# weimengmeng1999/AdapterSIS

Hardware: AMD Instinct MI355X
Metric: training images/sec, ViT-L/14 588^2 adapter fine-tune (higher is better)
Workload: dtype f16; 1 GPU; vit_large/14 frozen + CAViT/CACNN adapters (n_last_blocks=4) + FeatureDecoder, 588x588, batch 12/GPU, reference_exact train.py step (fwd + decoder bwd + all-reduce + SGD), random-init weights; global_batch=12, image_size=588, parallelism=dp1, split_precision_convs=True, split_attn_out=False, precise_level=0, fold_attn_scale=True, fused_qkv=False, dead_cacnn_elided=True, c1_elided=True, ln_fold=True, mx_conv=True, mx_dense=True, conv_halo=True, fuse_cls_up=False, skipped_optimizer_steps=0

## Files before the change

### adaptersis_amd/_lib.py

```python
from __future__ import annotations

import ctypes as C
import os

_HERE = os.path.dirname(os.path.abspath(__file__))
LIB_PATH = os.path.join(_HERE, "lib", "libasis_hip.so")

ASIS_F16, ASIS_BF16, ASIS_F32 = 0, 1, 2
ASIS_EINVAL, ASIS_ELAUNCH = -1, -2
ACT_NONE, ACT_GELU, ACT_RELU, ACT_SILU_MUL, ACT_GELU_GRAD = 0, 1, 2, 3, 4


class AsisError(RuntimeError):
    pass


class GemmDesc(C.Structure):
    _fields_ = [
        ("A", C.c_void_p), ("B", C.c_void_p), ("C", C.c_void_p),
        ("lda", C.c_int64), ("ldb", C.c_int64), ("ldc", C.c_int64),
        ("strideA", C.c_int64), ("strideB", C.c_int64), ("strideC", C.c_int64),
        ("batch", C.c_int32), ("M", C.c_int32), ("N", C.c_int32), ("K", C.c_int32),
        ("bias_n", C.c_void_p), ("bias_m", C.c_void_p), ("scale_n", C.c_void_p), ("res", C.c_void_p),
        ("ldr", C.c_int64), ("strideR", C.c_int64),
# ... 75 lines not shown
    "asis_dwconv_bwd_nblk": [_i64],
    "asis_dwconv_gelu_bwd": [_vp, _i, _vp, _vp, _vp, _vp, _vp, _i, _vp, _vp, _vp, _vp, _i, _i, _i],
    "asis_rowblock_nblk": [_i64],
    "asis_layernorm_bwd": [_vp, _vp, _i64, _vp, _i64, _vp, _f, _vp, _i64, _vp, _i64, _vp, _i64, _i],
    "asis_gelu16": [_vp, _i, _vp, _vp, _vp, _i64],
    "asis_gelu_split": [_vp, _i, _vp, _vp, _vp, _i64],
    "asis_cast_colsum": [_vp, _i, _vp, _i64, _vp, _i64, _f, _vp, _i64, _i],
    "asis_layernorm_gather": [_vp, _i, _vp, _i64, _vp, _vp, _f, _vp, _i64, _vp, _i, _i, _i64, _i],
    "asis_scaled_index_add": [_vp, _vp, _i64, _vp, _i64, _vp, _i64, _vp, _i, _i, _i64, _i],
    "asis_gather_cast_colsum": [_vp, _i, _vp, _i64, _vp, _i64, _vp, _vp, _i, _i, _i64, _i],
    "asis_layernorm_bwd_scatter": [_vp, _vp, _i64, _vp, _i64, _vp, _f, _vp, _i64, _vp, _i64, _vp, _vp, _i, _i, _i64, _i64, _i],
    "asis_swiglu_bwd": [_vp, _i, _vp, _vp, _vp, _i64, _i],
    "asis_colsum": [_vp, _i, _vp, _i64, _vp, _i64, _i],
    "asis_ls_linear_finish": [_vp, _vp, _vp, _vp, _vp, _vp, _f, _vp, _vp, _vp, _i, _i],
    "asis_attention_fwd": [_vp, _i, _vp, _vp, _i64, _vp, _i64, _vp, _i64, _i, _i, _i, _f],
    "asis_im2col_patch": [_vp, _i, _vp, _i, _i, _i, _i, _vp, _i64],
    "asis_im2col_patch_split": [_vp, _i, _vp, _i, _i, _i, _i, _vp, _vp, _i64],
    "asis_cast_pad": [_vp, _i, _vp, _i64, _vp, _i64, _i64, _i, _f, _i],
    "asis_add_cls_pos": [_vp, _vp, _vp, _vp, _vp, _i, _i, _i],
    "asis_msda_fwd": [_vp, _i, _vp, _vp, _i64, _vp, _vp, _vp, _vp, _i, _i, _i, _i, _i, _i, _i],
    "asis_msda_fwd_split": [_vp, _i, _vp, _vp, _i64, _vp, _vp, _vp, _vp, _vp, _i, _i, _i, _i, _i, _i, _i],
    "asis_dwconv_gelu": [_vp, _i, _vp, _vp, _vp, _vp, _vp, _i, _vp, _i, _i, _i],
    "asis_conv3x3_c3": [_vp, _vp, _vp, _vp, _i, _i, _i, _i, _i, _i],
    "asis_conv3x3_smallcout_fwd": [_vp, _i, _vp, _vp, _vp, _vp, _vp, _i, _i, _i, _i, _i],
    "asis_conv3x3_smallcout_fwd_up": [_vp, _i, _vp, _vp, _vp, _vp, _vp, _vp, _i, _i, _i, _i, _i],
    "asis_conv3x3_smallcout_wgrad_up": [_vp, _i, _vp, _i, _vp, _vp, _vp, _vp, _i, _i, _i, _i, _i, _i],
    "asis_cls_lowres_nblk": [_i, _i, _i],
    "asis_cls_lowres_fwd": [_vp, _vp, _vp, _vp, _vp, _vp, _vp, _vp, _i, _i, _i, _i, _i],
    "asis_cls_lowres_bwd": [_vp, _i, _vp, _vp, _i, _vp, _vp, _vp, _vp, _vp, _vp, _vp, _vp, _vp, _i, _i, _i, _i, _i, _i],
    "asis_dgrad_lowres_nblk": [_i, _i, _i],
    "asis_dgrad_lowres_cap": [_i],
    "asis_dgrad_lowres_pack": [_vp, _i, _vp, _vp, _vp, _i, _i],
    "asis_dgrad_lowres": [_vp, _i, _vp, _vp, _vp, _vp, _vp, _vp, _vp, _vp, _vp, _vp, _vp, _i, _i, _i, _i, _i, _i],
    "asis_conv3x3_smallcout_dgrad": [_vp, _i, _vp, _vp, _i, _vp, _vp, _i, _i, _i, _i, _i],
    "asis_conv3x3_smallcout_wgrad": [_vp, _i, _vp, _i, _vp, _vp, _i, _i, _i, _i, _i, _i],
    "asis_colstats_nparts": [_i64],
    "asis_colstats": [_vp, _vp, _i64, _i, _vp],
    "asis_reduce_partials": [_vp, _vp, _i, _i, _vp],
    "asis_bn_finalize": [_vp, _vp, _d, _i, _vp, _vp, _f, _f, _vp, _vp, _vp, _vp, _vp, _vp, _vp],
    "asis_bn_eval_affine": [_vp, _vp, _vp, _vp, _vp, _f, _i, _vp, _vp],
    "asis_bn_act": [_vp, _i, _vp, _vp, _vp, _i, _vp, _vp, _i64, _i],
    "asis_bn_act_mx": [_vp, _i, _vp, _vp, _vp, _i, _vp, _vp, _vp, _i64, _i],
    "asis_bn_relu_maxpool": [_vp, _i, _vp, _vp, _vp, _vp, _vp, _i, _i, _i, _i],
    "asis_bn_relu_upsample": [_vp, _i, _vp, _vp, _vp, _vp, _vp, _i, _i, _i, _i, _i],
    "asis_pack_conv_weight": [_vp, _i, _vp, _vp, _i, _i, _i, _i, _i, _i64, _i],
    "asis_decoder_input": [_vp, _i, _vp, _i64, _vp, _i64, _vp, _i64, _vp, _vp, _i, _i, _i, _i, _i, _i],
    "asis_swiglu": [_vp, _i, _vp, _vp, _i64, _i],
    "asis_swiglu_split": [_vp, _i, _vp, _vp, _vp, _i64, _i],
    "asis_copy_channels": [_vp, _vp, _i64, _vp, _i64, _i64, _i64],
    "asis_add_f32": [_vp, _vp, _vp, _vp, _i64, _i, _i64, _i64, _i64],
    "asis_maxpool2_fwd": [_vp, _i, _vp, _vp, _vp, _vp, _vp, _i, _i, _i, _i],
    "asis_maxpool2_bwd": [_vp, _vp, _vp, _vp, _i, _i, _i, _i],
    "asis_cls_l2norm": [_vp, _vp, _vp, _vp, _i, _i, _i, _i],
    "asis_cls_l2norm_bwd": [_vp, _vp, _vp, _vp, _vp, _i, _i, _i, _i],
    "asis_mask_logits_fwd": [_vp, _vp, _vp, _vp, _vp, _f, _vp, _vp, _vp, _i, _i, _i, _i],
    "asis_mask_logits_nblk": [_i, _i],
    "asis_mask_logits_bwd": [_vp, _vp, _vp, _vp, _vp, _vp, _vp, _f, _vp, _vp, _vp, _i, _i, _i, _i],
    "asis_mask_dchat": [_vp, _vp, _vp, _vp, _vp, _i, _i, _i, _i],
    "asis_nearest_add_relu": [_vp, _i, _vp, _vp, _vp, _vp, _vp, _vp, _i, _i, _i, _i, _i, _i],
    "asis_nearest_sum": [_vp, _vp, _vp, _vp, _vp, _i, _i, _i, _i, _i, _i],
    "asis_convt2x2_scatter": [_vp, _i, _vp, _vp, _vp, _i, _i, _i, _i, _i, _i, _i, _i, _i, _i],
    "asis_convt2x2_gather": [_vp, _i, _vp, _vp, _vp, _i, _i, _i, _i, _i, _i, _i, _i, _i, _i],
    "asis_convt2x2_bias_nblk": [_i64],
    "asis_conv1x1_dgrad_small": [_vp, _i, _vp, _vp, _i64, _vp, _vp, _i64, _i, _i],
    "asis_convt2x2_bias_grad": [_vp, _vp, _vp, _i, _i, _i, _i, _i, _i, _i, _i, _i, _i],
    "asis_dice_nblk": [_i, _i],
# ... 86 lines not shown
```

### adaptersis_amd/backbones/decoders.py

```python
from __future__ import annotations

import os
from typing import Dict, List, Optional

import torch
import torch.nn as nn
import torch.nn.functional as F

from .. import config, ops, parallel
from ..dinov2.layers.blocks import _Packed, _pack
from . import _bn


_DGRAD_MX = __import__("os").environ.get("ASIS_DGRAD_MX", "1") not in ("0", "")


class _Stage:
    __slots__ = ("x16", "raw", "scale", "shift", "mean", "invstd", "count", "factor", "stride", "pad", "pool", "cls_lowres", "dgrad_lowres")


def _conv_weights(owner: _Packed, key: str, conv: nn.Conv2d, split: bool):
    dt = config.operand_dtype
    if split:
        w_hi, w_lo, _ = _pack(owner._cache, key + ".wpair", conv.weight, lambda p: ops.pack_conv_weight_pair(p.float().contiguous(), 0, dt))
        return w_hi, w_lo
    return _pack(owner._cache, key + ".w", conv.weight, lambda p: ops.pack_conv_weight(p.float().contiguous(), 0, dt)), None


_KSPLIT = os.environ.get("ASIS_CONV_KSPLIT", "1") != "0"


def _conv_ksplit(P: int, Cout: int, Cin: int, split: bool) -> int:
    if not _KSPLIT or Cin % 64 or P < 256 or Cout < 32 or Cout % 4:
        return 1
    cus = 256
    plan = ops.conv3x3_plan(P, Cout, Cin, split)
    if plan and plan[0].startswith("conv_ph8"):
        tiles = plan[1]
        now, cut = -(-tiles // cus), -(-3 * tiles // cus) / 3.0 * 1.08
        return 3 if cut < 0.88 * now else 1
    tiles = ((P + 255) // 256) * ((Cout + 127) // 128 if Cout > 64 else (Cout + 63) // 64)

    def cost(t):
        c = -(-t // cus)
        return 1.7 * (c // 2) + (c % 2)

    now, cut = cost(tiles), cost(3 * tiles) / 3.0 * 1.08
    r = 3 if cut < 0.88 * now else 1
    if r == 3 and os.environ.get("ASIS_CONV_KSPLIT_DEBUG"):
        print(f"[ksplit] P={P} Cout={Cout} Cin={Cin} tiles={tiles} now={now:.2f} cut={cut:.2f}", flush=True)
    return r


def _conv_weights_mx(owner: _Packed, key: str, conv: nn.Conv2d):
    dt = config.operand_dtype
    amax = _w_amax(owner, key, conv)
    return _pack(owner._cache, key + ".wpairmx", conv.weight,
                 lambda p: ops.pack_conv_weight_pair(p.float().contiguous(), 0, dt, mx=True, amax=amax))


def _w_amax(owner: _Packed, key: str, conv: nn.Conv2d):
    return _pack(owner._cache, key + ".wamax", conv.weight, lambda p: ops.conv_weight_absmax(p.float().contiguous()))


def conv_bn_relu_up_forward(owner: _Packed, key: str, x16, x_lo, conv: nn.Conv2d, bn: nn.BatchNorm2d, factor: int,
                            sync_bn: bool, save: bool, training: bool = True, stride: int = 1, pad: int = 1,
                            pool: bool = False, mx_out: bool = False, defer_up: bool = False):
    dt = config.operand_dtype
    split_out = x_lo is not None
    if key in config.unsplit_layers:
        x_lo = None
    split = x_lo is not None
    B, H, W, _ = x16.shape
    OH, OW = (H + 2 * pad - 3) // stride + 1, (W + 2 * pad - 3) // stride + 1
    mx_in = ops.mx_amax_of(x_lo) if split else None
    if mx_in is not None:
        w_hi, w_lo, w_amax = _conv_weights_mx(owner, key, conv)
    else:
        w_hi, w_lo = _conv_weights(owner, key, conv, split)
    bias = owner._f32(key + ".b", conv.bias)
    ks = _conv_ksplit(B * OH * OW, conv.out_channels, x16.shape[3], split)
    stats = torch.empty((ops.gemm_tiles_m(B * OH * OW), 2, conv.out_channels), device=x16.device,
                        dtype=torch.float32) if (training and ks == 1) else None
    if mx_in is not None and ks == 1 and ops.conv_halo_ok(x16, conv.out_channels, stride, pad):
        raw = ops.conv3x3_halo_mx(x16, x_lo, w_hi, w_lo, (mx_in, w_amax), bias_n=bias, want_stats=training)
        if training:
            raw, stats = raw
    elif mx_in is not None:
        raw = ops.conv_gemm_split(x16, x_lo, w_hi, w_lo, 3, 3, stride, pad, bias_n=bias, stats=stats, ksplit=ks, mx=(mx_in, w_amax))
    elif split:
        raw = ops.conv_gemm_split(x16, x_lo, w_hi, w_lo, 3, 3, stride, pad, bias_n=bias, stats=stats, ksplit=ks)
    else:
        raw = ops.conv_gemm(x16, w_hi, 3, 3, stride, pad, bias_n=bias, stats=stats, ksplit=ks)
    if training and ks > 1:
        stats = ops.colstats(raw)
    if training:
        scale, shift, mean, invstd, count = _bn.finalize(stats, B * OH * OW, bn, sync_bn)
    else:
        scale, shift = ops.bn_eval_affine(bn)
        mean = invstd = count = None
        save = False
    if defer_up:
        up = ("deferred", raw, scale, shift)
    elif pool:
        up = ops.bn_relu_maxpool(raw, scale, shift, dt, split_out)
    elif factor > 1 and mx_out and split_out:
        up = ops.bn_relu_upsample(raw, scale, shift, factor, dt, True, mx_amax=ops.bn_relu_absmax(raw, scale, shift))
    elif factor > 1:
        up = ops.bn_relu_upsample(raw, scale, shift, factor, dt, split_out)
    elif mx_out and split_out:
        up = ops.bn_act(raw, scale, shift, True, dt, True, mx_amax=ops.bn_relu_absmax(raw, scale, shift))
    else:
        up = ops.bn_act(raw, scale, shift, True, dt, split_out)
    if not split_out and not defer_up:
        up = (up, None)
    st = None
    if save:
        st = _Stage()
        st.x16, st.raw, st.scale, st.shift, st.mean, st.invstd, st.count, st.factor = \
            x16, raw, scale, shift, mean, invstd, count, factor
        st.stride, st.pad, st.pool = stride, pad, pool
    return up, st


def conv_bn_relu_up_backward(owner: _Packed, key: str, st: _Stage, dU, conv: nn.Conv2d, bn: nn.BatchNorm2d,
                             inv_scale: float, grads: Dict[str, torch.Tensor], prefix: str, need_dx: bool,
                             sync_bn: bool, conv_name: Optional[str] = None, bn_name: Optional[str] = None,
                             lower: Optional[_Stage] = None):
    conv_name = conv_name or prefix + ".0"
    bn_name = bn_name or prefix + ".1"
    import torch.distributed as dist
    dt = config.operand_dtype
    C = conv.out_channels
    stride, pad = getattr(st, "stride", 1) or 1, getattr(st, "pad", 1)
    if isinstance(dU, tuple):
        g, partial = dU
    elif getattr(st, "pool", False):
        g, partial = ops.maxpool_bn_relu_bwd(dU, st.raw, st.scale, st.shift, st.mean, st.invstd)
    else:
        g, partial = ops.upsample_bn_relu_bwd(dU, st.raw, st.scale, st.shift, st.mean, st.invstd, st.factor)
    red = ops.reduce_rows(partial.view(partial.shape[0], 2 * C))
    local = red
    if sync_bn and parallel.bn_collectives_on():
        local = red.clone()
        dist.all_reduce(red)
    dbeta_s, dgamma_s = red[:C], red[C:]
    split = config.split_conv and need_dx
# ... 74 lines not shown
            parallel.join_grad_streams()
        return (None, None) + tuple(grads[n] for n in ctx.names)


class FeatureDecoder(_Packed):
    def __init__(self, img_size=588, inplanes=64, embed_dim=1024, num_classes=2, features=[1024, 512, 256, 128, 64]):
        super().__init__()
        self.img_size, self.features, self.inplanes = img_size, list(features), inplanes
        self.embed_dim, self.num_classes = embed_dim, num_classes
        chans = [features[0] * 3, features[1], features[2], features[3], features[4]]
        for c in chans:
            if c % 8:
                raise ValueError("FeatureDecoder channel counts must be multiples of 8")
        for i in range(4):
            setattr(self, f"decoder_{i + 1}", nn.Sequential(
                nn.Conv2d(chans[i], chans[i + 1], 3, padding=1), nn.BatchNorm2d(chans[i + 1]), nn.ReLU(inplace=True),
                nn.Upsample(scale_factor=2, mode="bilinear", align_corners=True)))
        self.final_out = nn.Conv2d(chans[4], num_classes, 3, padding=1)
        self.sync_bn = False

    GRAD_ORDER = ("final_out", "decoder_4", "decoder_3", "decoder_2", "decoder_1")

    def _to_nhwc16(self, x):
        B, C, H, W = x.shape
        x2 = x.detach().permute(0, 2, 3, 1).contiguous().float().view(B * H * W, C)
        hi = ops.cast_pad(x2, C, config.operand_dtype).view(B, H, W, C)
        lo = ops.cast_pad(x2, C, config.operand_dtype, part=1).view(B, H, W, C) if config.split_conv else None
        return hi, lo

    def _forward_core(self, x16, x_lo, save: bool, training: Optional[bool] = None):
        training = self.training if training is None else training
        saved: List = []
        a = (x16, x_lo)
        for i in range(1, 5):
            seq = getattr(self, f"decoder_{i}")
            nxt = getattr(self, f"decoder_{i + 1}")[0] if i < 4 else None
            Bq, Hq, Wq, _ = a[0].shape
            mx_out = bool(config.mx_conv_on() and a[1] is not None and nxt is not None and f"d{i + 1}" not in config.unsplit_layers and
                          ops.mx_conv_ok(Bq * 4 * Hq * Wq, nxt.in_channels, nxt.out_channels))
            fo = self.final_out
            fuse = bool(i == 4 and a[1] is not None and ops.FUSE_CLS_UP and seq[0].out_channels == 64 and fo.in_channels == 64 and
                        fo.out_channels <= 8 and Hq >= 4 and Wq >= 8)
            lowres = bool(i == 4 and not fuse and ops.CLS_LOWRES and seq[0].out_channels == 64 and fo.in_channels == 64 and
                          2 <= fo.out_channels <= 4 and Hq >= 2 and Wq >= 2)
            defer = fuse or lowres
            a, st = conv_bn_relu_up_forward(self, f"d{i}", a[0], a[1], seq[0], seq[1], 2, self.sync_bn, save, training, mx_out=mx_out,
                                            defer_up=defer)
            if lowres and st is not None:
                st.cls_lowres = True
            saved.append(st)
        if isinstance(a[0], str):
            if lowres:
                logits = ops.cls_lowres_fwd(a[1], a[2], a[3], self._f32("final.wf", self.final_out.weight),
                                            self._f32("final.b", self.final_out.bias))
            else:
                logits = ops.conv3x3_smallcout_fwd_up(a[1], a[2], a[3], self._f32("final.wf", self.final_out.weight),
                                                      self._f32("final.b", self.final_out.bias), config.operand_dtype)
            saved.append(None)
            return logits, saved
        logits = self._final_forward(a)
        saved.append(a[0] if save else None)
        return logits, saved

    def _final_forward(self, a):
        bias = self._f32("final.b", self.final_out.bias)
        fo = self.final_out
        if fo.out_channels <= 16 and fo.in_channels in (8, 16, 32, 64):
            return ops.conv3x3_smallcout_fwd(a[0], a[1], self._f32("final.wf", fo.weight), bias)
        w_hi, w_lo = _conv_weights(self, "final", self.final_out, a[1] is not None)
        if a[1] is not None:
            return ops.conv_gemm_split(a[0], a[1], w_hi, w_lo, 3, 3, 1, 1, bias_n=bias)
        return ops.conv_gemm(a[0], w_hi, 3, 3, 1, 1, bias_n=bias)

    def _final_backward(self, x5, d16, d_lo, bias_partial, inv_scale, grads, dlogits_f32, st4=None):
        C = self.num_classes
        if bias_partial is not None:
            ops.reduce_rows(bias_partial, inv_scale, grads["final_out.bias"])
        else:
            ops.reduce_rows(dlogits_f32, 1.0, grads["final_out.bias"])
        wout = grads["final_out.weight"]
        if x5 is None and getattr(st4, "cls_lowres", False):
            g, partial, slabs = ops.cls_lowres_bwd(d16, d_lo, st4.raw, st4.scale, st4.shift, st4.mean, st4.invstd,
                                                   self._f32("final.wf", self.final_out.weight), reduce=False)
# ... 314 lines not shown
```

### adaptersis_amd/config.py

```python
import os

import torch

operand_dtype = torch.bfloat16 if os.environ.get("ASIS_OPERAND", "f16").lower() in ("bf16", "bfloat16") else torch.float16
loss_scale = float(os.environ.get("ASIS_LOSS_SCALE", 65536.0 if operand_dtype == torch.float16 else 1.0))


def set_operand_dtype(dt: torch.dtype) -> None:
    global operand_dtype
    if dt not in (torch.float16, torch.bfloat16):
        raise ValueError("operand dtype must be float16 or bfloat16")
    operand_dtype = dt

split_conv = os.environ.get("ASIS_SPLIT_CONV", "1") != "0"

precise_attention = os.environ.get("ASIS_PRECISE", "0") not in ("0", "")
fold_attn_scale = os.environ.get("ASIS_FOLD_SCALE", "1") not in ("0", "")
fused_qkv = os.environ.get("ASIS_FUSED_QKV", "0") not in ("0", "")

encoder_stream = os.environ.get("ASIS_ENC_STREAM", "1") not in ("0", "")

vt_stream = os.environ.get("ASIS_VT_STREAM", "1") not in ("0", "")

wgrad_stream = os.environ.get("ASIS_WGRAD_STREAM", "1") not in ("0", "")
# ... 33 lines not shown

_mx = os.environ.get("ASIS_MX_CONV", "1")
mx_conv_all = _mx == "2"
mx_conv = _mx not in ("0", "")


def mx_conv_on() -> bool:
    return mx_conv and (mx_conv_all or operand_dtype == torch.float16)


mx_dense = os.environ.get("ASIS_MX_DENSE", "1") not in ("0", "")


def mx_dense_on() -> bool:
    return mx_dense and operand_dtype == torch.float16

_DGRAD_LOWRES_ALL = ("d2", "d3", "d4")


def parse_dgrad_lowres(v: str) -> frozenset:
    v = (v or "").strip().lower()
    if v in ("", "0"):
        return frozenset()
    if v == "1":
        return frozenset(_DGRAD_LOWRES_ALL)
    keys = [k.strip() for k in v.split(",") if k.strip()]
    bad = [k for k in keys if k not in _DGRAD_LOWRES_ALL]
    if bad:
        raise ValueError(f"ASIS_DGRAD_LOWRES={v!r}: expected 0, 1 or a list of {', '.join(_DGRAD_LOWRES_ALL)} (unknown: {', '.join(bad)})")
    return frozenset(keys)


dgrad_lowres = parse_dgrad_lowres(os.environ.get("ASIS_DGRAD_LOWRES", "1"))
```

### adaptersis_amd/csrc/core.hip

```cpp
#include <stdarg.h>

#include "asis_common.h"

static thread_local char g_err[512] = "";

extern "C" void asis_set_error_(const char* fmt, ...) {
  va_list ap;
  va_start(ap, fmt);
  vsnprintf(g_err, sizeof(g_err), fmt, ap);
  va_end(ap);
}

extern "C" const char* asis_last_error(void) { return g_err; }
extern "C" int asis_version(void) { return 100; }

extern "C" int asis_device_count(void) {
  int n = 0;
  hipError_t e = hipGetDeviceCount(&n);
  if (e != hipSuccess) {
    asis_set_error_("hipGetDeviceCount: %s", hipGetErrorString(e));
    (void)hipGetLastError();
    return ASIS_ELAUNCH;
  }
  return n;
}
```

### adaptersis_amd/ops.py

```python
from __future__ import annotations

import ctypes as C
import functools
import os
from typing import Optional

import torch

from . import _lib, config
from ._lib import ACT_GELU, ACT_GELU_GRAD, ACT_NONE, ACT_RELU, ACT_SILU_MUL, GemmDesc, check, lib

T16_DEFAULT = torch.float16

PROFILE = None


def _launch_timed(kind: str, flops: float, fn, nbytes: float = 0.0):
    if PROFILE is None:
        return fn()
    s, e = torch.cuda.Event(enable_timing=True), torch.cuda.Event(enable_timing=True)
    s.record()
    rc = fn()
    e.record()
    PROFILE.append((kind, flops, s, e, nbytes))
# ... 833 lines not shown

def dgrad_lowres_pack(w: torch.Tensor, dtype: torch.dtype):
    _dev(w)
    Co, Ck = w.shape[0], w.shape[1]
    if w.dtype != torch.float32 or not w.is_contiguous() or tuple(w.shape[2:]) != (3, 3):
        raise ValueError("dgrad_lowres_pack: contiguous float32 [Co, Ck, 3, 3] expected")
    hi = torch.empty((max(Co // 16, 1), 5, Ck, 32), device=w.device, dtype=dtype)
    lo = torch.empty_like(hi)
    check(lib().asis_dgrad_lowres_pack(_stream(), _dt(dtype), w.data_ptr(), hi.data_ptr(), lo.data_ptr(), Co, Ck),
          "asis_dgrad_lowres_pack")
    return hi, lo


def dgrad_lowres(d16: torch.Tensor, d_lo: Optional[torch.Tensor], wpack, raw: torch.Tensor, scale, shift, mean, invstd):
    _dev(d16, d_lo, raw)
    _not_mx("dgrad_lowres", d_lo)
    B, H, W, Ck = raw.shape
    Co = d16.shape[3]
    w_hi, w_lo = wpack
    if not d16.is_contiguous() or tuple(d16.shape[:3]) != (B, 2 * H, 2 * W) or (d_lo is not None and
                                                                                 (d_lo.shape != d16.shape or not d_lo.is_contiguous())):
        raise ValueError("dgrad_lowres: d16 / d_lo must be contiguous [B, 2H, 2W, Co]")
    if raw.dtype != torch.float32 or not raw.is_contiguous() or w_hi.dtype != d16.dtype or w_hi.numel() != (Co // 16) * 5 * Ck * 32:
        raise ValueError("dgrad_lowres: raw must be contiguous float32 [B, H, W, Ck] and the weight pack that of a [Co, Ck, 3, 3] conv")
    nblk = lib().asis_dgrad_lowres_nblk(B, H, W)
    g = torch.empty_like(raw)
    partial = torch.empty((nblk, 2, Ck), device=raw.device, dtype=torch.float32)
    check(lib().asis_dgrad_lowres(_stream(), _dt(d16.dtype), d16.data_ptr(), _p(d_lo), w_hi.data_ptr(), w_lo.data_ptr(), raw.data_ptr(),
                                  _f32c(scale).data_ptr(), _f32c(shift).data_ptr(), _f32c(mean).data_ptr(), _f32c(invstd).data_ptr(),
                                  g.data_ptr(), partial.data_ptr(), nblk, B, H, W, Co, Ck), "asis_dgrad_lowres")
    return g, partial


def conv3x3_smallcout_dgrad(dy_hi: torch.Tensor, dy_lo: Optional[torch.Tensor], w: torch.Tensor) -> torch.Tensor:
    _dev(dy_hi, dy_lo, w)
    B, H, W, CoP = dy_hi.shape
    Cout, Cin = w.shape[0], w.shape[1]
    dx = torch.empty((B, H, W, Cin), device=dy_hi.device, dtype=torch.float32)
    check(lib().asis_conv3x3_smallcout_dgrad(_stream(), _dt(dy_hi.dtype), dy_hi.data_ptr(), _p(dy_lo), CoP,
                                             _f32c(w).data_ptr(), dx.data_ptr(), B, H, W, Cin, Cout),
          "asis_conv3x3_smallcout_dgrad")
    return dx


def colstats(x: torch.Tensor) -> torch.Tensor:
    _dev(x)
    Cc = x.shape[-1]
    R = x.numel() // Cc
    nparts = lib().asis_colstats_nparts(R)
    partial = torch.empty((nparts, 2, Cc), device=x.device, dtype=torch.float32)
    check(lib().asis_colstats(_stream(), _f32c(x).data_ptr(), R, Cc, partial.data_ptr()), "asis_colstats")
    return partial


def reduce_partials(partial: torch.Tensor) -> torch.Tensor:
    _dev(partial)
    nparts, _, Cc = partial.shape
    sums = torch.empty((2, Cc), device=partial.device, dtype=torch.float64)
    check(lib().asis_reduce_partials(_stream(), _f32c(partial).data_ptr(), nparts, Cc, sums.data_ptr()),
          "asis_reduce_partials")
    return sums


def bn_finalize(sums: torch.Tensor, count: float, gamma, beta, eps: float, momentum: float, running_mean=None,
                running_var=None, num_batches_tracked=None):
    _dev(sums, gamma, beta, running_mean, running_var, num_batches_tracked)
# ... 1604 lines not shown
```

### include/asis_hip.h

```cpp
#ifndef ASIS_HIP_H
#define ASIS_HIP_H

#include <stdint.h>

#ifdef __cplusplus
extern "C" {
#endif

#define ASIS_OK 0
#define ASIS_EINVAL (-1)
#define ASIS_ELAUNCH (-2)

#define ASIS_F16 0
#define ASIS_BF16 1
#define ASIS_F32 2

#define ASIS_ACT_NONE 0
#define ASIS_ACT_GELU 1
#define ASIS_ACT_RELU 2
#define ASIS_ACT_SILU_MUL 3
#define ASIS_ACT_GELU_GRAD 4

const char* asis_last_error(void);
int asis_version(void);
// ... 131 lines not shown
                              const int32_t* shapes, const int32_t* starts, void* ST, int64_t ldt, int B, int Lq, int Lin,
                              int M, int L, int P);
int asis_dwconv_bwd_nblk(int64_t rows);
int asis_dwconv_gelu_bwd(void* stream, int dtype, const float* x, const float* w9, const float* bias, const int32_t* shapes,
                         const int32_t* starts, int L, const float* dy, float* g, float* partial, void* dx, int B, int Ntok,
                         int C);

int asis_conv3x3_c3(void* stream, const float* img, const float* w, float* out, int B, int H, int W, int Cout,
                    int stride, int pad);
int asis_conv3x3_smallcout_fwd(void* stream, int dtype, const void* x_hi, const void* x_lo, const float* w,
                               const float* bias, float* out, int B, int H, int W, int Cin, int Cout);
int asis_conv3x3_smallcout_dgrad(void* stream, int dtype, const void* dy_hi, const void* dy_lo, int CoP, const float* w,
                                 float* dx, int B, int H, int W, int Cin, int Cout);

int asis_conv3x3_smallcout_fwd_up(void* stream, int dtype, const float* raw, const float* scale, const float* shift, const float* w,
                                  const float* bias, float* out, int B, int H, int W, int Cin, int Cout);
int asis_conv3x3_smallcout_wgrad_up(void* stream, int dtype, const void* dy, int CoP, const float* raw, const float* scale,
                                    const float* shift, float* slabs, int nblk, int B, int H, int W, int Cin, int Cout);

int asis_cls_lowres_nblk(int B, int H, int W);
int asis_cls_lowres_fwd(void* stream, const float* raw, const float* scale, const float* shift, const float* w, const float* bias,
                        float* z, float* out, int B, int H, int W, int Cin, int Cout);
int asis_cls_lowres_bwd(void* stream, int dtype, const void* d16, const void* d_lo, int CoP, const float* raw, const float* scale,
                        const float* shift, const float* mean, const float* invstd, const float* w, float* g, float* partial,
                        float* slabs, int nblk, int B, int H, int W, int Cin, int Cout);

int asis_dgrad_lowres_nblk(int B, int H, int W);
int asis_dgrad_lowres_cap(int cap);
int asis_dgrad_lowres_pack(void* stream, int dtype, const float* w, void* w_hi, void* w_lo, int Co, int Ck);
int asis_dgrad_lowres(void* stream, int dtype, const void* d16, const void* d_lo, const void* w_hi, const void* w_lo, const float* raw,
                      const float* scale, const float* shift, const float* mean, const float* invstd, float* g, float* partial,
                      int nblk, int B, int H, int W, int Co, int Ck);

int asis_conv3x3_smallcout_wgrad(void* stream, int dtype, const void* dy, int CoP, const void* x, float* slabs, int nblk,
                                 int B, int H, int W, int Cin, int Cout);
int asis_colstats_nparts(int64_t R);
int asis_colstats(void* stream, const float* x, int64_t R, int C, float* partial);
int asis_reduce_partials(void* stream, const float* partial, int nparts, int C, double* sums);
int asis_bn_finalize(void* stream, const double* sums, double count, int C, const float* gamma, const float* beta,
                     float eps, float momentum, float* running_mean, float* running_var, int64_t* num_batches_tracked,
                     float* scale, float* shift, float* mean_out, float* invstd_out);
int asis_bn_eval_affine(void* stream, const float* gamma, const float* beta, const float* running_mean,
                        const float* running_var, float eps, int C, float* scale, float* shift);
int asis_bn_act(void* stream, int dtype, const float* x, const float* scale, const float* shift, int relu, void* out,
                void* out_lo, int64_t R, int C);
int asis_bn_act_mx(void* stream, int dtype, const float* x, const float* scale, const float* shift, int relu, void* out, void* out_mx,
                   const float* amax, int64_t R, int C);
int asis_bn_relu_maxpool(void* stream, int dtype, const float* x, const float* scale, const float* shift, void* out,
                         void* out_lo, int B, int H, int W, int C);
int asis_bn_relu_upsample(void* stream, int dtype, const float* x, const float* scale, const float* shift, void* out,
                          void* out_lo, int B, int H, int W, int C, int factor);
int asis_bn_relu_upsample_mx(void* stream, int dtype, const float* x, const float* scale, const float* shift, void* out,
                             void* out_mx, const float* amax, int B, int H, int W, int C, int factor);
int asis_pack_conv_weight(void* stream, int dtype, const float* w, void* out, int Cout, int Cin, int KH, int KW,
                          int mode, int64_t ldo, int part);
int asis_pack_conv_weight_mx(void* stream, int dtype, const float* w, void* out_mx, int Cout, int Cin, int KH, int KW,
                             int mode, int64_t ldo, const float* amax);
int asis_pack_conv_weight_pair(void* stream, int dtype, const float* w, void* out_hi, void* out_lo, int Cout, int Cin, int KH,
                               int KW, int mode, int64_t ldo, const float* amax);
int asis_decoder_input(void* stream, int dtype, const float* xs, int64_t xs_bstride, const float* c4,
                       int64_t c4_bstride, const float* vit, int64_t vit_bstride, void* out, void* out_lo, int B, int h,
                       int w, int h4, int w4, int D);
int asis_decoder_input_mx(void* stream, int dtype, const float* xs, int64_t xs_bstride, const float* c4, int64_t c4_bstride,
                          const float* vit, int64_t vit_bstride, void* out, void* out_mx, const float* amax, int B, int h,
                          int w, int h4, int w4, int D);
int asis_swiglu(void* stream, int dtype, const float* x12, void* out, int64_t R, int Hd);
// ... 184 lines not shown
```

Baseline: 232.1 img/s.

## Run decoder conv at low resolution before bilinear upsample for d2/d3

For decoder stages d2 and d3, the 3x3 conv no longer runs on the 2x bilinearly upsampled map. Instead the previous stage emits its low-resolution BN+ReLU output, a split-precision GEMM computes all 9 taps at low resolution into a [B,H,W,9,Co] buffer, and a new gather kernel applies the align-corners bilinear upsample per tap, adds the bias and accumulates BN statistics. This cuts the conv GEMM work about fourfold and avoids materialising the upsampled input. The cost is a large fp32 intermediate of 9*Co values per low-res pixel, plus an upsampled copy still built when activations are saved for backward. Zero-padding at the high-res borders is handled by skipping out-of-range taps.

```diff
diff --git a/adaptersis_amd/_lib.py b/adaptersis_amd/_lib.py
--- a/adaptersis_amd/_lib.py
+++ b/adaptersis_amd/_lib.py
@@ -131,6 +131,9 @@
     "asis_dgrad_lowres_cap": [_i],
     "asis_dgrad_lowres_pack": [_vp, _i, _vp, _vp, _vp, _i, _i],
     "asis_dgrad_lowres": [_vp, _i, _vp, _vp, _vp, _vp, _vp, _vp, _vp, _vp, _vp, _vp, _vp, _i, _i, _i, _i, _i, _i],
+    "asis_conv_lowres_tiles": [_i, _i, _i],
+    "asis_conv_lowres_pack": [_vp, _i, _vp, _vp, _vp, _i, _i],
+    "asis_conv_lowres_gather": [_vp, _vp, _vp, _vp, _vp, _i, _i, _i, _i, _i],
     "asis_conv3x3_smallcout_dgrad": [_vp, _i, _vp, _vp, _i, _vp, _vp, _i, _i, _i, _i, _i],
     "asis_conv3x3_smallcout_wgrad": [_vp, _i, _vp, _i, _vp, _vp, _i, _i, _i, _i, _i, _i],
     "asis_colstats_nparts": [_i64],
diff --git a/adaptersis_amd/backbones/decoders.py b/adaptersis_amd/backbones/decoders.py
--- a/adaptersis_amd/backbones/decoders.py
+++ b/adaptersis_amd/backbones/decoders.py
@@ -16,7 +16,7 @@
 
 
 class _Stage:
-    __slots__ = ("x16", "raw", "scale", "shift", "mean", "invstd", "count", "factor", "stride", "pad", "pool", "cls_lowres", "dgrad_lowres")
+    __slots__ = ("x16", "raw", "scale", "shift", "mean", "invstd", "count", "factor", "stride", "pad", "pool", "cls_lowres", "dgrad_lowres", "conv_lowres")
 
 
 def _conv_weights(owner: _Packed, key: str, conv: nn.Conv2d, split: bool):
@@ -65,8 +65,20 @@
 
 def conv_bn_relu_up_forward(owner: _Packed, key: str, x16, x_lo, conv: nn.Conv2d, bn: nn.BatchNorm2d, factor: int,
                             sync_bn: bool, save: bool, training: bool = True, stride: int = 1, pad: int = 1,
-                            pool: bool = False, mx_out: bool = False, defer_up: bool = False):
+                            pool: bool = False, mx_out: bool = False, defer_up: bool = False, low_out: bool = False):
     dt = config.operand_dtype
+    if isinstance(x16, tuple):
+        _, y_hi, y_lo = x16
+        x16 = x_lo
+        wp = _pack(owner._cache, key + ".wlowres", conv.weight, lambda p: ops.conv_lowres_pack(p.float().contiguous(), dt))
+        raw = ops.conv_lowres_fwd(y_hi, y_lo, wp, owner._f32(key + ".b", conv.bias), want_stats=training)
+        stats = None
+        if training:
+            raw, stats = raw
+        up, st = _bn_relu_out(raw, stats, x16, True, bn, factor, sync_bn, save, training, 1, 1, False, mx_out, defer_up, low_out)
+        if st is not None:
+            st.conv_lowres = True
+        return up, st
     split_out = x_lo is not None
     if key in config.unsplit_layers:
         x_lo = None
@@ -94,14 +106,23 @@
         raw = ops.conv_gemm(x16, w_hi, 3, 3, stride, pad, bias_n=bias, stats=stats, ksplit=ks)
     if training and ks > 1:
         stats = ops.colstats(raw)
+    return _bn_relu_out(raw, stats, x16, split_out, bn, factor, sync_bn, save, training, stride, pad, pool, mx_out, defer_up, low_out)
+
+
+def _bn_relu_out(raw, stats, x16, split_out: bool, bn: nn.BatchNorm2d, factor: int, sync_bn: bool, save: bool, training: bool,
+                 stride: int, pad: int, pool: bool, mx_out: bool, defer_up: bool, low_out: bool):
+    dt = config.operand_dtype
     if training:
-        scale, shift, mean, invstd, count = _bn.finalize(stats, B * OH * OW, bn, sync_bn)
+        scale, shift, mean, invstd, count = _bn.finalize(stats, raw.numel() // raw.shape[3], bn, sync_bn)
     else:
         scale, shift = ops.bn_eval_affine(bn)
         mean = invstd = count = None
         save = False
     if defer_up:
         up = ("deferred", raw, scale, shift)
+    elif low_out:
+        y_hi, y_lo = ops.bn_act(raw, scale, shift, True, dt, True)
+        up = (("lowres", y_hi, y_lo), ops.bn_relu_upsample(raw, scale, shift, factor, dt, False) if save else None)
     elif pool:
         up = ops.bn_relu_maxpool(raw, scale, shift, dt, split_out)
     elif factor > 1 and mx_out and split_out:
@@ -112,7 +133,7 @@
         up = ops.bn_act(raw, scale, shift, True, dt, True, mx_amax=ops.bn_relu_absmax(raw, scale, shift))
     else:
         up = ops.bn_act(raw, scale, shift, True, dt, split_out)
-    if not split_out and not defer_up:
+    if not split_out and not defer_up and not low_out:
         up = (up, None)
     st = None
     if save:
@@ -253,23 +274,28 @@
         training = self.training if training is None else training
         saved: List = []
         a = (x16, x_lo)
+        split = x_lo is not None
+        Bq, Hq, Wq, _ = x16.shape
         for i in range(1, 5):
             seq = getattr(self, f"decoder_{i}")
             nxt = getattr(self, f"decoder_{i + 1}")[0] if i < 4 else None
-            Bq, Hq, Wq, _ = a[0].shape
-            mx_out = bool(config.mx_conv_on() and a[1] is not None and nxt is not None and f"d{i + 1}" not in config.unsplit_layers and
+            mx_out = bool(config.mx_conv_on() and split and nxt is not None and f"d{i + 1}" not in config.unsplit_layers and
                           ops.mx_conv_ok(Bq * 4 * Hq * Wq, nxt.in_channels, nxt.out_channels))
             fo = self.final_out
-            fuse = bool(i == 4 and a[1] is not None and ops.FUSE_CLS_UP and seq[0].out_channels == 64 and fo.in_channels == 64 and
+            fuse = bool(i == 4 and split and ops.FUSE_CLS_UP and seq[0].out_channels == 64 and fo.in_channels == 64 and
                         fo.out_channels <= 8 and Hq >= 4 and Wq >= 8)
             lowres = bool(i == 4 and not fuse and ops.CLS_LOWRES and seq[0].out_channels == 64 and fo.in_channels == 64 and
                           2 <= fo.out_channels <= 4 and Hq >= 2 and Wq >= 2)
             defer = fuse or lowres
-            a, st = conv_bn_relu_up_forward(self, f"d{i}", a[0], a[1], seq[0], seq[1], 2, self.sync_bn, save, training, mx_out=mx_out,
-                                            defer_up=defer)
+            low_out = bool(nxt is not None and split and f"d{i + 1}" not in config.unsplit_layers and
+                           ops.conv_lowres_on(f"d{i + 1}") and nxt.in_channels == seq[0].out_channels and
+                           ops.conv_lowres_ok(nxt.out_channels, nxt.in_channels, Hq, Wq))
+            a, st = conv_bn_relu_up_forward(self, f"d{i}", a[0], a[1], seq[0], seq[1], 2, self.sync_bn, save, training,
+                                            mx_out=mx_out and not low_out, defer_up=defer, low_out=low_out)
             if lowres and st is not None:
                 st.cls_lowres = True
             saved.append(st)
+            Hq, Wq = 2 * Hq, 2 * Wq
         if isinstance(a[0], str):
             if lowres:
                 logits = ops.cls_lowres_fwd(a[1], a[2], a[3], self._f32("final.wf", self.final_out.weight),
diff --git a/adaptersis_amd/config.py b/adaptersis_amd/config.py
--- a/adaptersis_amd/config.py
+++ b/adaptersis_amd/config.py
@@ -89,3 +89,21 @@
 
 
 dgrad_lowres = parse_dgrad_lowres(os.environ.get("ASIS_DGRAD_LOWRES", "1"))
+
+_CONV_LOWRES_DEFAULT = ("d2", "d3")
+
+
+def parse_conv_lowres(v: str) -> frozenset:
+    v = (v or "").strip().lower()
+    if v in ("", "0"):
+        return frozenset()
+    if v == "1":
+        return frozenset(_CONV_LOWRES_DEFAULT)
+    keys = [k.strip() for k in v.split(",") if k.strip()]
+    bad = [k for k in keys if k not in _DGRAD_LOWRES_ALL]
+    if bad:
+        raise ValueError(f"ASIS_CONV_LOWRES={v!r}: expected 0, 1 or a list of {', '.join(_DGRAD_LOWRES_ALL)} (unknown: {', '.join(bad)})")
+    return frozenset(keys)
+
+
+conv_lowres = parse_conv_lowres(os.environ.get("ASIS_CONV_LOWRES", "1"))
diff --git a/adaptersis_amd/csrc/convlowres.hip b/adaptersis_amd/csrc/convlowres.hip
--- /dev/null
+++ b/adaptersis_amd/csrc/convlowres.hip
@@ -0,0 +1,204 @@
+#include "asis_common.h"
+
+namespace {
+
+constexpr int TY = 16, TX = 16;
+constexpr int WR = TY / 2 + 3, WC = TX / 2 + 3;
+constexpr int CC = 16;
+constexpr int NT = 512;
+constexpr int NQ = WR * WC * 9 * (CC / 4);
+constexpr int NPF = (NQ + NT - 1) / NT;
+constexpr size_t LDS_BYTES = (size_t)NQ * 16;
+
+__device__ __forceinline__ void tap_ac_true(int o, float r, int in, int& i0, int& i1, float& l0, float& l1) {
+  const float s = r * (float)o;
+  i0 = (int)s;
+  i1 = i0 + ((i0 < in - 1) ? 1 : 0);
+  l1 = s - (float)i0;
+  l0 = 1.f - l1;
+}
+
+template <typename T>
+__global__ __launch_bounds__(256) void conv_lowres_pack_kernel(const float* __restrict__ w, T* __restrict__ hi, T* __restrict__ lo,
+                                                               int Co, int Ck, int64_t total) {
+  for (int64_t o = (int64_t)blockIdx.x * 256 + threadIdx.x; o < total; o += (int64_t)gridDim.x * 256) {
+    const int k = (int)(o % Ck);
+    const int64_t r = o / Ck;
+    const int co = (int)(r % Co), tap = (int)(r / Co);
+    const float v = w[((int64_t)co * Ck + k) * 9 + tap];
+    hi[o] = to_t16<T>(v);
+    lo[o] = to_t16<T>(lo_part<T>(v));
+  }
+}
+
+template <bool STATS>
+__global__ __launch_bounds__(NT) void conv_lowres_gather_kernel(const float* __restrict__ z, const float* __restrict__ bias,
+                                                                float* __restrict__ out, float* __restrict__ stats, int H, int W, int Co,
+                                                                int tiles_x, int tiles_y, int nch, int nwork) {
+  extern __shared__ __attribute__((aligned(16))) float win[];
+  const int t = threadIdx.x;
+  const int work = xcd_remap(blockIdx.x, gridDim.x);
+  if (work >= nwork) return;
+  const int tile = work / nch, ch0 = (work - tile * nch) * CC;
+  const int b = tile / (tiles_x * tiles_y), tr = tile - b * (tiles_x * tiles_y);
+  const int y0 = (tr / tiles_x) * TY, x0 = (tr % tiles_x) * TX;
+  const int OH = 2 * H, OW = 2 * W;
+  const float rh = (float)(H - 1) / (float)(OH - 1), rw = (float)(W - 1) / (float)(OW - 1);
+  const int i_lo = (int)(rh * (float)(y0 > 0 ? y0 - 1 : 0)), j_lo = (int)(rw * (float)(x0 > 0 ? x0 - 1 : 0));
+  const int cg = t & 3;
+  const bool cok = ch0 + 4 * cg < Co;
+
+  {
+    const float* zb = z + (int64_t)b * H * W * 9 * Co + ch0 + 4 * cg;
+    float4 v[NPF];
+#pragma unroll
+    for (int r = 0; r < NPF; ++r) {
+      const int it = t + NT * r, q = it >> 2, px = q / 9, tap = q - px * 9;
+      const int wr = px / WC, i = i_lo + wr, j = j_lo + (px - wr * WC);
+      v[r] = make_float4(0.f, 0.f, 0.f, 0.f);
+      if (it < NQ && cok && i < H && j < W) v[r] = *reinterpret_cast<const float4*>(zb + ((int64_t)(i * W + j) * 9 + tap) * Co);
+    }
+#pragma unroll
+    for (int r = 0; r < NPF; ++r) {
+      const int it = t + NT * r;
+      if (it < NQ) reinterpret_cast<float4*>(win)[it] = v[r];
+    }
+  }
+  __syncthreads();
+
+  const int p = t >> 2, tx = p & 15, ty = p >> 4;
+  const int x = x0 + tx;
+  int xo0[3], xo1[3];
+  float xl0[3], xl1[3];
+  bool xok[3];
+#pragma unroll
+  for (int d = 0; d < 3; ++d) {
+    const int X = x + d - 1;
+    xok[d] = (unsigned)X < (unsigned)OW;
+    int a0, a1;
+    tap_ac_true(xok[d] ? X : 0, rw, W, a0, a1, xl0[d], xl1[d]);
+    xo0[d] = (a0 - j_lo) * 9 * CC;
+    xo1[d] = (a1 - j_lo) * 9 * CC;
+  }
+  float4 bv = make_float4(0.f, 0.f, 0.f, 0.f);
+  if (bias && cok) bv = *reinterpret_cast<const float4*>(bias + ch0 + 4 * cg);
+  float4 s1 = make_float4(0.f, 0.f, 0.f, 0.f), s2 = s1;
+#pragma unroll
+  for (int pp = 0; pp < 2; ++pp) {
+    const int y = y0 + ty + 8 * pp;
+    if (y < OH && x < OW && cok) {
+      float4 acc = bv;
+#pragma unroll
+      for (int ky = 0; ky < 3; ++ky) {
+        const int Y = y + ky - 1;
+        if ((unsigned)Y >= (unsigned)OH) continue;
+        int a0, a1;
+        float yl0, yl1;
+        tap_ac_true(Y, rh, H, a0, a1, yl0, yl1);
+        const float* r0 = win + (a0 - i_lo) * (WC * 9 * CC) + ky * 3 * CC + 4 * cg;
+        const float* r1 = win + (a1 - i_lo) * (WC * 9 * CC) + ky * 3 * CC + 4 * cg;
+#pragma unroll
+        for (int kx = 0; kx < 3; ++kx) {
+          if (!xok[kx]) continue;
+          const float4 v00 = *reinterpret_cast<const float4*>(r0 + xo0[kx] + kx * CC);
+          const float4 v01 = *reinterpret_cast<const float4*>(r0 + xo1[kx] + kx * CC);
+          const float4 v10 = *reinterpret_cast<const float4*>(r1 + xo0[kx] + kx * CC);
+          const float4 v11 = *reinterpret_cast<const float4*>(r1 + xo1[kx] + kx * CC);
+          const float w00 = yl0 * xl0[kx], w01 = yl0 * xl1[kx], w10 = yl1 * xl0[kx], w11 = yl1 * xl1[kx];
+#define ASIS_BLEND(c) acc.c += __fmaf_rn(w11, v11.c, __fmaf_rn(w10, v10.c, __fmaf_rn(w01, v01.c, w00 * v00.c)))
+          ASIS_BLEND(x); ASIS_BLEND(y); ASIS_BLEND(z); ASIS_BLEND(w);
+#undef ASIS_BLEND
+        }
+      }
+      *reinterpret_cast<float4*>(out + (((int64_t)b * OH + y) * OW + x) * Co + ch0 + 4 * cg) = acc;
+      if constexpr (STATS) {
+        s1.x += acc.x; s1.y += acc.y; s1.z += acc.z; s1.w += acc.w;
+        s2.x += acc.x * acc.x; s2.y += acc.y * acc.y; s2.z += acc.z * acc.z; s2.w += acc.w * acc.w;
+      }
+    }
+  }
+
+  if constexpr (STATS) {
+#pragma unroll
+    for (int o = 4; o < 64; o <<= 1) {
+      s1.x += __shfl_xor(s1.x, o, 64); s1.y += __shfl_xor(s1.y, o, 64); s1.z += __shfl_xor(s1.z, o, 64); s1.w += __shfl_xor(s1.w, o, 64);
+      s2.x += __shfl_xor(s2.x, o, 64); s2.y += __shfl_xor(s2.y, o, 64); s2.z += __shfl_xor(s2.z, o, 64); s2.w += __shfl_xor(s2.w, o, 64);
+    }
+    __syncthreads();
+    const int lane = t & 63, wave = t >> 6;
+    if (lane < 4) {
+      *reinterpret_cast<float4*>(win + (wave * 2 + 0) * CC + 4 * lane) = s1;
+      *reinterpret_cast<float4*>(win + (wave * 2 + 1) * CC + 4 * lane) = s2;
+    }
+    __syncthreads();
+    if (t < 2 * CC) {
+      const int q = t / CC, c = t - q * CC;
+      if (ch0 + c < Co) {
+        float s = 0.f;
+#pragma unroll
+        for (int wv = 0; wv < NT / 64; ++wv) s += win[(wv * 2 + q) * CC + c];
+        stats[((int64_t)tile * 2 + q) * Co + ch0 + c] = s;
+      }
+    }
+  }
+}
+
+template <bool STATS> int set_lds() {
+  return hipFuncSetAttribute(reinterpret_cast<const void*>(&conv_lowres_gather_kernel<STATS>), hipFuncAttributeMaxDynamicSharedMemorySize,
+                             (int)LDS_BYTES) != hipSuccess;
+}
+
+}
+
+extern "C" int asis_conv_lowres_tiles(int B, int H, int W) {
+  if (B < 1 || H < 1 || W < 1) return 0;
+  const int64_t n = (int64_t)B * ((2 * (int64_t)H + TY - 1) / TY) * ((2 * (int64_t)W + TX - 1) / TX);
+  return n < (1 << 30) ? (int)n : 0;
+}
+
+extern "C" int asis_conv_lowres_pack(void* stream, int dtype, const float* w, void* w_hi, void* w_lo, int Co, int Ck) {
+  ASIS_REQUIRE(w && w_hi && w_lo, "asis_conv_lowres_pack: null pointer");
+  ASIS_REQUIRE(Co >= 1 && Ck >= 1 && (int64_t)Co * Ck * 9 < (1ll << 31), "asis_conv_lowres_pack: bad shape Co=%d Ck=%d", Co, Ck);
+  ASIS_DT_OK(dtype, "asis_conv_lowres_pack");
+  const int64_t total = (int64_t)9 * Co * Ck;
+  if (int rc = asis_dispatch16(dtype, "asis_conv_lowres_pack", [&](auto t) {
+        using T = decltype(t);
+        hipLaunchKernelGGL((conv_lowres_pack_kernel<T>), dim3(asis_grid(total, 256, 2048)), dim3(256), 0,
+                           reinterpret_cast<hipStream_t>(stream), w, static_cast<T*>(w_hi), static_cast<T*>(w_lo), Co, Ck, total);
+      })) return rc;
+  ASIS_CHECK_LAUNCH("asis_conv_lowres_pack");
+  return ASIS_OK;
+}
+
+extern "C" int asis_conv_lowres_gather(void* stream, const float* z, const float* bias, float* out, float* stats, int ntiles, int B,
+                                       int H, int W, int Co) {
+  ASIS_REQUIRE(z && out, "asis_conv_lowres_gather: null pointer");
+  ASIS_REQUIRE(B > 0 && H >= 2 && W >= 2 && H < (1 << 24) && W < (1 << 24), "asis_conv_lowres_gather: the map %d x %d x %d must be at least 2 x 2",
+               B, H, W);
+  ASIS_REQUIRE(Co >= 4 && Co % 4 == 0 && Co <= 4096, "asis_conv_lowres_gather: Co=%d must be a multiple of 4, at most 4096", Co);
+  ASIS_REQUIRE((int64_t)H * W * 9 * Co < (1ll << 31), "asis_conv_lowres_gather: %d x %d x 9 x %d: one image of z must stay below 2^31 values",
+               H, W, Co);
+  ASIS_REQUIRE(ntiles > 0 && ntiles == asis_conv_lowres_tiles(B, H, W), "asis_conv_lowres_gather: ntiles=%d, asis_conv_lowres_tiles gives %d",
+               ntiles, asis_conv_lowres_tiles(B, H, W));
+  ASIS_REQUIRE(asis_aligned16(z) && asis_aligned16(out) && (!bias || asis_aligned16(bias)) && (!stats || asis_aligned16(stats)),
+               "asis_conv_lowres_gather: alignment");
+  const int tx = (2 * W + TX - 1) / TX, ty = (2 * H + TY - 1) / TY, nch = (Co + CC - 1) / CC;
+  const int64_t nw = (int64_t)ntiles * nch;
+  ASIS_REQUIRE(nw < (1ll << 31), "asis_conv_lowres_gather: too many workgroups");
+  hipStream_t s = reinterpret_cast<hipStream_t>(stream);
+  int bad;
+  if (stats) {
+    bad = set_lds<true>();
+    if (!bad)
+      hipLaunchKernelGGL((conv_lowres_gather_kernel<true>), dim3((unsigned)nw), dim3(NT), LDS_BYTES, s, z, bias, out, stats, H, W, Co, tx, ty,
+                         nch, (int)nw);
+  } else {
+    bad = set_lds<false>();
+    if (!bad)
+      hipLaunchKernelGGL((conv_lowres_gather_kernel<false>), dim3((unsigned)nw), dim3(NT), LDS_BYTES, s, z, bias, out, stats, H, W, Co, tx, ty,
+                         nch, (int)nw);
+  }
+  if (bad) ASIS_FAIL(ASIS_ELAUNCH, "asis_conv_lowres_gather: %zu bytes of LDS refused", LDS_BYTES);
+  ASIS_CHECK_LAUNCH("asis_conv_lowres_gather");
+  return ASIS_OK;
+}
diff --git a/adaptersis_amd/csrc/core.hip b/adaptersis_amd/csrc/core.hip
--- a/adaptersis_amd/csrc/core.hip
+++ b/adaptersis_amd/csrc/core.hip
@@ -12,7 +12,7 @@
 }
 
 extern "C" const char* asis_last_error(void) { return g_err; }
-extern "C" int asis_version(void) { return 100; }
+extern "C" int asis_version(void) { return 101; }
 
 extern "C" int asis_device_count(void) {
   int n = 0;
diff --git a/adaptersis_amd/ops.py b/adaptersis_amd/ops.py
--- a/adaptersis_amd/ops.py
+++ b/adaptersis_amd/ops.py
@@ -889,6 +889,58 @@
     return g, partial
 
 
+CONV_LOWRES = config.conv_lowres
+
+
+def conv_lowres_on(key: str) -> bool:
+    return bool(CONV_LOWRES) if isinstance(CONV_LOWRES, bool) else key in CONV_LOWRES
+
+
+def conv_lowres_ok(Co: int, Ck: int, H: int, W: int) -> bool:
+    return bool(Ck >= 64 and Ck % 64 == 0 and Co >= 8 and Co % 8 == 0 and Co <= 4096 and H >= 2 and W >= 2 and H * W * 9 * Co < (1 << 31))
+
+
+def conv_lowres_weight_matrix(w: torch.Tensor) -> torch.Tensor:
+    Co, Ck = w.shape[0], w.shape[1]
+    return w.permute(2, 3, 0, 1).reshape(9 * Co, Ck)
+
+
+def conv_lowres_pack(w: torch.Tensor, dtype: torch.dtype):
+    _dev(w)
+    if w.dtype != torch.float32 or not w.is_contiguous() or w.dim() != 4 or tuple(w.shape[2:]) != (3, 3):
+        raise ValueError("conv_lowres_pack: contiguous float32 [Co, Ck, 3, 3] expected")
+    Co, Ck = w.shape[0], w.shape[1]
+    hi = torch.empty((9 * Co, Ck), device=w.device, dtype=dtype)
+    lo = torch.empty_like(hi)
+    check(lib().asis_conv_lowres_pack(_stream(), _dt(dtype), w.data_ptr(), hi.data_ptr(), lo.data_ptr(), Co, Ck), "asis_conv_lowres_pack")
+    return hi, lo
+
+
+def conv_lowres_gather(z: torch.Tensor, bias: Optional[torch.Tensor], want_stats: bool = False):
+    _dev(z, bias)
+    if z.dtype != torch.float32 or not z.is_contiguous() or z.dim() != 5 or z.shape[3] != 9:
+        raise ValueError("conv_lowres_gather: z must be contiguous float32 [B, H, W, 9, Co]")
+    B, H, W, _, Co = z.shape
+    ntiles = lib().asis_conv_lowres_tiles(B, H, W)
+    out = torch.empty((B, 2 * H, 2 * W, Co), device=z.device, dtype=torch.float32)
+    stats = torch.empty((ntiles, 2, Co), device=z.device, dtype=torch.float32) if want_stats else None
+    check(lib().asis_conv_lowres_gather(_stream(), z.data_ptr(), _p(_f32c(bias)), out.data_ptr(), _p(stats), ntiles, B, H, W, Co),
+          "asis_conv_lowres_gather")
+    return (out, stats) if want_stats else out
+
+
+def conv_lowres_fwd(y_hi: torch.Tensor, y_lo: torch.Tensor, wpack, bias: Optional[torch.Tensor], want_stats: bool = False):
+    _not_mx("conv_lowres_fwd", y_lo)
+    w_hi, w_lo = wpack
+    B, H, W, Ck = y_hi.shape
+    Co = w_hi.shape[0] // 9
+    if not (y_hi.is_contiguous() and y_lo.is_contiguous() and y_lo.shape == y_hi.shape and w_hi.shape[1] == Ck):
+        raise ValueError("conv_lowres_fwd: contiguous NHWC planes [B, H, W, Ck] and a [9 Co, Ck] weight pack expected")
+    z = torch.empty((B * H * W, 9 * Co), device=y_hi.device, dtype=torch.float32)
+    gemm_split(y_hi.view(B * H * W, Ck), y_lo.view(B * H * W, Ck), w_hi, w_lo, out=z)
+    return conv_lowres_gather(z.view(B, H, W, 9, Co), bias, want_stats)
+
+
 def conv3x3_smallcout_dgrad(dy_hi: torch.Tensor, dy_lo: Optional[torch.Tensor], w: torch.Tensor) -> torch.Tensor:
     _dev(dy_hi, dy_lo, w)
     B, H, W, CoP = dy_hi.shape
diff --git a/include/asis_hip.h b/include/asis_hip.h
--- a/include/asis_hip.h
+++ b/include/asis_hip.h
@@ -187,6 +187,11 @@
                       const float* scale, const float* shift, const float* mean, const float* invstd, float* g, float* partial,
                       int nblk, int B, int H, int W, int Co, int Ck);
 
+int asis_conv_lowres_tiles(int B, int H, int W);
+int asis_conv_lowres_pack(void* stream, int dtype, const float* w, void* w_hi, void* w_lo, int Co, int Ck);
+int asis_conv_lowres_gather(void* stream, const float* z, const float* bias, float* out, float* stats, int ntiles, int B, int H, int W,
+                            int Co);
+
 int asis_conv3x3_smallcout_wgrad(void* stream, int dtype, const void* dy, int CoP, const void* x, float* slabs, int nblk,
                                  int B, int H, int W, int Cin, int Cout);
 int asis_colstats_nparts(int64_t R);
```

Result: no change. 234.1 img/s (median of 6 runs) (+0.9%).
